# ska-telescope/ska-sdp-idg-bench

Hardware: AMD Instinct MI355X
Metric: Mvisibilities/s (gridder & degridder) at 1/2/4/8 GPUs; % HBM roofline (higher is better)
Workload: dtype f32 phase/accumulate, f16x2-split MFMA operands

## Files before the change

ska-sdp-idg-bench_amd/csrc/hip/kernels/gridder_mi355x.hip.cpp:

```cpp
#include <hip/hip_runtime.h>

#include <cstdlib>
#include <string>

#include "../util.hpp"
#include "device.hpp"
#include "fft.hpp"
#include "lib-hip.hpp"
#include "mfma.hpp"

#ifndef IDG_GRID_PT
#define IDG_GRID_PT 4
#endif
#ifndef IDG_GRID_WAVES
#define IDG_GRID_WAVES 4
#endif
#ifndef IDG_GRID_WAVES_GENERAL
#define IDG_GRID_WAVES_GENERAL 4
#endif
#ifndef IDG_GRID_BSCALE
#define IDG_GRID_BSCALE 12
#endif
#ifndef IDG_GRID_NW
#define IDG_GRID_NW 8
#endif

namespace idg_mi355x {

namespace {

__device__ __forceinline__ void mac4(float *a, const float4 &va,
                                     const float4 &vb, float cs, float sn) {
  a[0] = fma_(va.x, cs, a[0]); a[0] = fma_(-va.y, sn, a[0]);
  a[1] = fma_(va.x, sn, a[1]); a[1] = fma_(va.y, cs, a[1]);
  a[2] = fma_(va.z, cs, a[2]); a[2] = fma_(-va.w, sn, a[2]);
  a[3] = fma_(va.z, sn, a[3]); a[3] = fma_(va.w, cs, a[3]);
  a[4] = fma_(vb.x, cs, a[4]); a[4] = fma_(-vb.y, sn, a[4]);
  a[5] = fma_(vb.x, sn, a[5]); a[5] = fma_(vb.y, cs, a[5]);
  a[6] = fma_(vb.z, cs, a[6]); a[6] = fma_(-vb.w, sn, a[6]);
  a[7] = fma_(vb.z, sn, a[7]); a[7] = fma_(vb.w, cs, a[7]);
}

template <int NP, int CB>
__device__ __forceinline__ void timestep_general(
    const float (&l)[NP], const float (&m)[NP], const float (&n)[NP],
    const float (&poff)[NP], float (&acc)[NP][8],
    const idg::UVWCoordinate<float> c, const float4 *__restrict__ vrow,
    const float *__restrict__ wavenumbers, int C) {
  float pidx[NP];
#pragma unroll
  for (int i = 0; i < NP; ++i)
    pidx[i] = fma_(c.w, n[i], fma_(c.u, l[i], c.v * m[i]));
  for (int cb = 0; cb < C; cb += CB) {
    const int ce = min(cb + CB, C);
    const float k0 = wavenumbers[cb];
    float A[NP], R[NP];
#pragma unroll
    for (int i = 0; i < NP; ++i) {
      A[i] = fma_(-pidx[i], k0, poff[i]);
      R[i] = revolutions(A[i]);
    }
    float k = k0;
    float4 va = vrow[2 * cb], vb = vrow[2 * cb + 1];
    for (int ch = cb; ch < ce; ++ch) {
      const int nx = min(ch + 1, C - 1);
      const float kn = wavenumbers[nx];
      const float4 van = vrow[2 * nx], vbn = vrow[2 * nx + 1];
#pragma unroll
      for (int i = 0; i < NP; ++i) {
        const float ph = fma_(-pidx[i], k, poff[i]);
        const float r = fma_(ph - A[i], kInv2PiHi, R[i]);
        float sn, cs;
        sincos_rev(r, &sn, &cs);
        mac4(acc[i], va, vb, cs, sn);
      }
      k = kn;
      va = van;
      vb = vbn;
    }
  }
}

template <int NB, int CB>
__device__ __forceinline__ void timestep_mirror(
    const float (&l)[2 * NB], const float (&m)[2 * NB],
    const float (&poff)[2 * NB], float (&acc)[2 * NB][8],
    const idg::UVWCoordinate<float> c, const float4 *__restrict__ vrow,
    const float *__restrict__ wavenumbers, int C) {
  float pidx[NB];
#pragma unroll
  for (int i = 0; i < NB; ++i) pidx[i] = fma_(c.u, l[i], c.v * m[i]);
  for (int cb = 0; cb < C; cb += CB) {
    const int ce = min(cb + CB, C);
    const float k0 = wavenumbers[cb];
    float A[NB], R[NB];
#pragma unroll
    for (int i = 0; i < NB; ++i) {
      A[i] = fma_(-pidx[i], k0, poff[i]);
      R[i] = revolutions(A[i]);
    }
    float k = k0;
    float4 va = vrow[2 * cb], vb = vrow[2 * cb + 1];
    for (int ch = cb; ch < ce; ++ch) {
      const int nx = min(ch + 1, C - 1);
      const float kn = wavenumbers[nx];
      const float4 van = vrow[2 * nx], vbn = vrow[2 * nx + 1];
#pragma unroll
      for (int i = 0; i < NB; ++i) {
        const float ph = fma_(-pidx[i], k, poff[i]);
        const float r = fma_(ph - A[i], kInv2PiHi, R[i]);
        float sn, cs;
        sincos_rev(r, &sn, &cs);
        mac4(acc[i], va, vb, cs, sn);
        mac4(acc[NB + i], va, vb, cs, -sn);
      }
      k = kn;
      va = van;
      vb = vbn;
    }
  }
}

__device__ __forceinline__ void pixel_out(const float (&a)[8], int p, int S,
                                          const SubgridSetup &g,
                                          int nr_stations,
                                          const float *__restrict__ spheroidal,
                                          const float2 *__restrict__ aterms,
                                          float2 (&o)[4]) {
  const int y = p / S, x = p - (p / S) * S;
  idg::cfloat pix[4], a1[4], a2[4];
  for (int q = 0; q < 4; ++q) pix[q] = {a[2 * q], a[2 * q + 1]};
  load_jones(aterm_ptr(aterms, nr_stations, S, g.aterm_index, g.station1, y,
                       x), a1);
  load_jones(aterm_ptr(aterms, nr_stations, S, g.aterm_index, g.station2, y,
                       x), a2);
  idg::apply_aterm_gridder(pix, a1, a2);
  const float sph = spheroidal[p];
#pragma unroll
  for (int q = 0; q < 4; ++q) o[q] = make_float2(pix[q].re * sph, pix[q].im * sph);
}

__device__ __forceinline__ void store_pixel(
    const float (&a)[8], int p, int S, int npix, const SubgridSetup &g,
    int nr_stations, const float *__restrict__ spheroidal,
    const float2 *__restrict__ aterms, float2 *__restrict__ out) {
  float2 o[4];
  pixel_out(a, p, S, g, nr_stations, spheroidal, aterms, o);
#pragma unroll
  for (int q = 0; q < 4; ++q) out[static_cast<size_t>(q) * npix + p] = o[q];
}

template <bool W_TERMS = true>
__device__ __forceinline__ void pixel_geometry(int p, int S, float image_size,
                                               const SubgridSetup &g,
                                               float &l, float &m, float &n,
                                               float &poff) {
  const int y = p / S, x = p - (p / S) * S;
  l = idg::compute_l(x, S, image_size);
  m = idg::compute_m(y, S, image_size);
  if constexpr (W_TERMS) {
    n = idg::compute_n(l, m);
    poff = fma_(g.w_offset, n, fma_(g.u_offset, l, g.v_offset * m));
  } else {
    n = 0.0f;
    poff = fma_(g.u_offset, l, g.v_offset * m);
  }
}


#ifndef IDG_GRID_KSBUF
#define IDG_GRID_KSBUF 32
#endif
constexpr int kKsBuf = IDG_GRID_KSBUF;
#ifndef IDG_GRID_KSBUF_MIRROR
#define IDG_GRID_KSBUF_MIRROR (2 * IDG_GRID_KSBUF)
#endif
constexpr int kKsBufMirror = IDG_GRID_KSBUF_MIRROR;
#ifndef IDG_GRID_FILL_DEPTH
#define IDG_GRID_FILL_DEPTH 2
#endif
constexpr int mirror_fill_depth(int S_CT, bool combined) {
  return combined && S_CT != 32 ? 1 : IDG_GRID_FILL_DEPTH;
}

template <int AT, int NW>
struct MfmaLds {
  static constexpr int kObufFloats = NW * 16 * AT * 16;
  static constexpr int kBbufWords = kKsBuf * 64 * 8;
  static_assert(kKsBufMirror * 64 * 4 <= kBbufWords, "one buffer, two layouts");
  static constexpr int kUvwOff =
      kObufFloats > kBbufWords ? kObufFloats : kBbufWords;
  static constexpr int kRedOff = kUvwOff + 4 * 4 * kKsBuf;
  static constexpr int kSlotOff = kRedOff + 8;
  static constexpr int kSinkOff = kSlotOff + 2;
  static constexpr int kWords = kSinkOff + 64;
  static constexpr int kGeoOff = kWords;
  static constexpr int kWordsGeo = kGeoOff + 64 + 2 * 1024;
};
template <int S_CT, int NW, int AT>
constexpr int general_lds_words() {
  return S_CT == 32 ? MfmaLds<AT, NW>::kWordsGeo : MfmaLds<AT, NW>::kWords;
}

__device__ __forceinline__ void l2_prefetch_dma(const void *src,
                                                const void *lds_dst) {
  const unsigned m0 = __builtin_amdgcn_readfirstlane(static_cast<unsigned>(
      reinterpret_cast<size_t>((const __attribute__((address_space(3))) void *)
                                   lds_dst)));
  unsigned saved;
  asm volatile(
      "s_mov_b32 %0, m0\n\ts_mov_b32 m0, %2\n\ts_nop 0\n\t"
      "global_load_lds_dword %1, off\n\ts_mov_b32 m0, %0"
      : "=&s"(saved)
      : "v"(src), "s"(m0)
      : "memory");
}

template <int S_CT, int PT, int CB, int NW, bool MIRROR, bool FFT = false,
          int PREC = kPrecTail, bool PRESCAN = false,
          int FILL_D = IDG_GRID_FILL_DEPTH>
__device__ __forceinline__ void grid_mfma(
    const SubgridSetup &g, int S, int npix, float image_size, int C,
    int nr_stations, const idg::UVWCoordinate<float> *__restrict__ uvw,
    const float *__restrict__ wavenumbers,
    const float2 *__restrict__ visibilities,
    const float *__restrict__ spheroidal, const float2 *__restrict__ aterms,
    float2 *__restrict__ out, unsigned *lds, float vmax_pre = 0.0f,
    int pass_lo = 0, int pass_hi = 1 << 30) {
  static_assert(CB % 4 == 0, "anchor blocks hold whole channel quads");
  int tid = threadIdx.x;
  if constexpr (!MIRROR) asm volatile("" : "+v"(tid));
  const int lane = tid & 63, wave = tid >> 6;
  const int grp = lane >> 4, col = lane & 15;
  const int half = MIRROR ? npix / 2 : npix;
  constexpr bool kTailAlt = (PREC & kPrecTailAlt) != 0;
  constexpr bool kTailAll = (PREC & kPrecTail) != 0 && !kTailAlt;
  constexpr int AT = MIRROR ? 2 * PT : PT;
  using Lds = MfmaLds<AT, NW>;
  constexpr bool kGeoLds = !MIRROR && S_CT == 32;
  float *geo = reinterpret_cast<float *>(lds + Lds::kGeoOff);
  const int nt = g.nr_timesteps;
  const int nchq = (C + 3) / 4;
  const int nquads = (nt + 3) / 4;
  constexpr bool kOneFrag = MIRROR && S_CT != 0;
  constexpr int KS = kOneFrag ? kKsBufMirror : kKsBuf;
  const int quads_per_fill = nchq <= KS ? min(KS / nchq, kKsBuf) : 1;
  const int cq_per_fill = nchq <= KS ? nchq : KS;
  unsigned *slots = lds + Lds::kSlotOff;

  float vmax = vmax_pre;
  if (tid < 2) slots[tid] = 0u;
  if constexpr (!PRESCAN) {
    vmax = 0.0f;
    const float4 *v4 = reinterpret_cast<const float4 *>(
        visibilities + g.time_offset * C * 4);
    const int n4 = min(4 * quads_per_fill, nt) * C * 2;
    for (int i = tid; i < n4; i += NW * 64) {
      const float4 q = v4[i];
      vmax = fmaxf(vmax, fmaxf(fmaxf(fabsf(q.x), fabsf(q.y)),
                               fmaxf(fabsf(q.z), fabsf(q.w))));
    }
    for (int off = 32; off > 0; off >>= 1)
      vmax = fmaxf(vmax, __shfl_xor(vmax, off));
    float *red = reinterpret_cast<float *>(lds + Lds::kRedOff);
    if (lane == 0) red[wave] = vmax;
    __syncthreads();
#pragma unroll
    for (int w = 0; w < NW; ++w) vmax = fmaxf(vmax, red[w]);
  }
  constexpr int kBS = IDG_GRID_BSCALE;
  static_assert(kBS >= 0 && kBS <= 14, "a fill may reach 2^15 before it re-splits");
  int e = 0;
  bool have_scale = vmax > 0.0f && vmax <= 3.0e38f;
  if (have_scale) frexpf(vmax, &e);
  float scale = ldexpf(1.0f, kBS - e);
  int fidx = 0;

  const float2 *__restrict__ vsub = visibilities + g.time_offset * C * 4;

  uint4 *bbuf = reinterpret_cast<uint4 *>(lds);
  float *obuf = reinterpret_cast<float *>(lds);
  float4 *tuvw = reinterpret_cast<float4 *>(lds + Lds::kUvwOff);

  constexpr int kPass = NW * 16 * PT;
  for (int gbase = pass_lo; gbase < min(half, pass_hi); gbase += kPass) {
    static_assert(PT % 2 == 0, "phases are packed over tile pairs");
    constexpr int PH = PT / 2;
    floatx2 L2[PH], M2[PH], N2[PH], PG2[PH];
    if constexpr (kGeoLds) {
      static_assert(PT == 8 && NW == 8, "one S = 32 pass: 1,024 pixels");
      for (int p = tid; p < 1024; p += NW * 64) {
        float l, m, n, pg;
        pixel_geometry<true>(p, 32, image_size, g, l, m, n, pg);
        geo[64 + p] = n;
        geo[64 + 1024 + p] = pg;
        if (p < 32) geo[p] = l;
        if (p % 32 == 0) geo[32 + p / 32] = m;
      }
    } else {
#pragma unroll
      for (int i = 0; i < PT; ++i) {
        const int b = min(gbase + (wave * PT + i) * 16 + col, half - 1);
        float l, m, n, pg;
        pixel_geometry<!MIRROR>(b, S, image_size, g, l, m, n, pg);
        L2[i / 2][i % 2] = l;
        M2[i / 2][i % 2] = m;
        N2[i / 2][i % 2] = n;
        PG2[i / 2][i % 2] = pg;
      }
    }
    constexpr int PY = MIRROR ? PT : 1;
    floatx4 accx[PT], accy[PY];
#pragma unroll
    for (int i = 0; i < PT; ++i) accx[i] = floatx4{0.0f, 0.0f, 0.0f, 0.0f};
#pragma unroll
    for (int i = 0; i < PY; ++i) accy[i] = floatx4{0.0f, 0.0f, 0.0f, 0.0f};

    constexpr bool kFlush = (PREC & kPrecFlush) != 0;
    static_assert(!kFlush || S_CT == 32,
                  "the master fills the S = 32 output slot in one pass");
    bool flushed = false;
    auto master = [&](int t) {
      return reinterpret_cast<float4 *>(out) +
             ((wave * AT + t) * 32 + grp * 8 + (col & 7));
    };
    auto flush_tile = [&](floatx4 &a, int t, float unsc) {
      const float a0 = a[0], a1 = a[1], a2 = a[2], a3 = a[3];
      const float v0 = (a0 + row_ror8(a0)) * unsc;
      const float v1 = (a1 + row_ror8(a1)) * unsc;
      const float v2 = (a2 + row_ror8(a2)) * unsc;
      const float v3 = (a3 + row_ror8(a3)) * unsc;
      if (col < 8) {
        float4 m = make_float4(0.0f, 0.0f, 0.0f, 0.0f);
        if (flushed) m = *master(t);
        *master(t) = make_float4(m.x + v0, m.y + v1, m.z + v2, m.w + v3);
      }
      a = floatx4{0.0f, 0.0f, 0.0f, 0.0f};
    };

    for (int q0 = 0; q0 < nquads; q0 += quads_per_fill) {
      const int nq = min(quads_per_fill, nquads - q0);
      for (int j0 = 0; j0 < nchq; j0 += cq_per_fill, ++fidx) {
        const int nj = min(cq_per_fill, nchq - j0);
        for (;;) {
        __syncthreads();
        if (tid == 0) slots[(fidx + 1) & 1] = 0u;
        {
          const int bpol = (col & 7) >> 1;
          const int w_c = 2 * bpol + (col & 1);
          const int w_s = 2 * bpol + 1 - (col & 1);
          const float sc_s = (col & 1) ? scale : -scale;
          const float bpart = (col & 8) ? -1.0f : 0.0f;
          const float *vsubf = reinterpret_cast<const float *>(vsub);
          const int nks = nq * nj;
          const bool full = (q0 + nq) * 4 <= nt && 4 * (j0 + nj) <= C;
          const int wv = __builtin_amdgcn_readfirstlane(wave);
          const unsigned off_c = (grp * C * 8 + w_c) * 4u;
          const unsigned off_s = (grp * C * 8 + w_s) * 4u;
          int qq = wv / nj, jj = wv - (wv / nj) * nj;
          float lmax = 0.0f;
          if constexpr (kOneFrag) {
            auto load4 = [&](int q_, int j_, float (&b)[4]) {
              const int c0 = 4 * (j0 + j_);
              if (full) {
                const char *blk = reinterpret_cast<const char *>(
                    vsubf + ((q0 + q_) * 4 * C + c0) * 8);
#pragma unroll
                for (int u = 0; u < 4; ++u)
                  b[u] = *reinterpret_cast<const float *>(blk + off_c + 32 * u);
              } else {
                const int t = (q0 + q_) * 4 + grp;
#pragma unroll
                for (int u = 0; u < 4; ++u) {
                  const bool ok = t < nt && c0 + u < C;
                  b[u] = ok ? vsubf[(t * C + c0 + u) * 8 + w_c] : 0.0f;
                }
              }
            };
            auto put = [&](int ks, const float (&b)[4]) {
              lmax = fmaxf(lmax, fmaxf(fmaxf(fabsf(b[0]), fabsf(b[1])),
                                       fmaxf(fabsf(b[2]), fabsf(b[3]))));
              const unsigned xc =
                  split_part(b[0] * scale, b[1] * scale, bpart);
              const unsigned yc =
                  split_part(b[2] * scale, b[3] * scale, bpart);
              bbuf[ks * 64 + lane] = make_uint4(xc, xc, yc, yc);
            };
            auto advance = [&]() {
              jj += NW;
              while (jj >= nj) {
                jj -= nj;
                ++qq;
              }
            };
            constexpr int D = FILL_D;
            for (int ks = wv; ks < nks; ks += D * NW) {
              float b[D][4];
#pragma unroll
              for (int d = 0; d < D; ++d)
                if (ks + d * NW < nks) {
                  load4(qq, jj, b[d]);
                  advance();
                }
#pragma unroll
              for (int d = 0; d < D; ++d)
                if (ks + d * NW < nks) put(ks + d * NW, b[d]);
            }
          } else {
          for (int ks = wv; ks < nks; ks += NW) {
            const int t = (q0 + qq) * 4 + grp;
            const int c0 = 4 * (j0 + jj);
            float bc[4], bs[4];
            if (full) {
              const char *blk = reinterpret_cast<const char *>(
                  vsubf + ((q0 + qq) * 4 * C + c0) * 8);
#pragma unroll
              for (int u = 0; u < 4; ++u) {
                const float rc =
                    *reinterpret_cast<const float *>(blk + off_c + 32 * u);
                const float rs =
                    *reinterpret_cast<const float *>(blk + off_s + 32 * u);
                lmax = fmaxf(lmax, fmaxf(fabsf(rc), fabsf(rs)));
                bc[u] = rc * scale;
                bs[u] = rs * sc_s;
              }
            } else {
#pragma unroll
              for (int u = 0; u < 4; ++u) {
                const bool ok = t < nt && c0 + u < C;
                const int it = ok ? t * C + c0 + u : 0;
                const float rc = ok ? vsubf[it * 8 + w_c] : 0.0f;
                const float rs = ok ? vsubf[it * 8 + w_s] : 0.0f;
                lmax = fmaxf(lmax, fmaxf(fabsf(rc), fabsf(rs)));
                bc[u] = rc * scale;
                bs[u] = rs * sc_s;
              }
            }
            jj += NW;
            while (jj >= nj) {
              jj -= nj;
              ++qq;
            }
            const unsigned xc = split_part(bc[0], bc[1], bpart);
            const unsigned yc = split_part(bc[2], bc[3], bpart);
            const unsigned xs = split_part(bs[0], bs[1], bpart);
            const unsigned ys = split_part(bs[2], bs[3], bpart);
            bbuf[(ks * 64 + lane) * 2] = make_uint4(xc, xc, yc, yc);
            bbuf[(ks * 64 + lane) * 2 + 1] = make_uint4(xs, xs, ys, ys);
          }
          }
          {
            unsigned v = __float_as_uint(lmax);
            v = max(v, (unsigned)__builtin_amdgcn_update_dpp(0, (int)v, 0xB1, 0xF, 0xF, false));
            v = max(v, (unsigned)__builtin_amdgcn_update_dpp(0, (int)v, 0x4E, 0xF, 0xF, false));
            v = max(v, (unsigned)__builtin_amdgcn_update_dpp(0, (int)v, 0x124, 0xF, 0xF, false));
            v = max(v, (unsigned)__builtin_amdgcn_update_dpp(0, (int)v, 0x128, 0xF, 0xF, false));
            const unsigned wmax =
                max(max(__builtin_amdgcn_readlane(v, 0), __builtin_amdgcn_readlane(v, 16)),
                    max(__builtin_amdgcn_readlane(v, 32), __builtin_amdgcn_readlane(v, 48)));
            if (lane == 0) atomicMax(&slots[fidx & 1], wmax);
          }
          for (int i = tid; i < nq * 4; i += NW * 64) {
            const idg::UVWCoordinate<float> c =
                uvw[g.time_offset + min(q0 * 4 + i, nt - 1)];
            tuvw[i] = make_float4(c.u, c.v, c.w, 0.0f);
          }
        }
        __syncthreads();
        const float fm = __uint_as_float(
            __builtin_amdgcn_readfirstlane(slots[fidx & 1]));
        if (!(fm > 0.0f && fm <= 3.0e38f)) break;
        int em;
        frexpf(fm, &em);
        if (have_scale ? em <= e + 15 - kBS : em == e) {
          have_scale = true;
          break;
        }
        if (have_scale) {
          const float r = ldexpf(1.0f, e - em);
#pragma unroll
          for (int i = 0; i < PT; ++i) accx[i] *= r;
#pragma unroll
          for (int i = 0; i < PY; ++i) accy[i] *= r;
        }
        e = em;
        scale = ldexpf(1.0f, kBS - e);
        have_scale = true;
        }
        {
          int q0n = q0, j0n = j0 + cq_per_fill;
          if (j0n >= nchq) {
            j0n = 0;
            q0n = q0 + quads_per_fill;
          }
          if (q0n < nquads) {
            const int rows = min(4 * (q0n + quads_per_fill), nt) - 4 * q0n;
            const int lpr = (min(cq_per_fill, nchq - j0n) * 128 + 127) / 128;
            const char *vb = reinterpret_cast<const char *>(vsub);
            for (int ln = tid; ln < rows * lpr; ln += NW * 64) {
              const int row = ln / lpr, cl = ln - (ln / lpr) * lpr;
              l2_prefetch_dma(
                  vb + (static_cast<size_t>(4 * q0n + row) * C + 4 * j0n) * 32 +
                      cl * 128,
                  lds + Lds::kSinkOff);
            }
          }
        }
        for (int jb = 0; jb < nj; jb += CB / 4) {
          const int je = min(jb + CB / 4, nj);
          const float ka = wavenumbers[4 * (j0 + jb)];
          float kb[CB];
#pragma unroll
          for (int v = 0; v < CB; ++v)
            kb[v] = wavenumbers[min(4 * (j0 + jb) + v, C - 1)];
          for (int qq = 0; qq < nq; ++qq) {
            const float4 c4 = tuvw[qq * 4 + grp];
            const idg::UVWCoordinate<float> c = {c4.x, c4.y, c4.z};
            const floatx2 cu = {c.u, c.u}, cv = {c.v, c.v};
            const floatx2 ih = {kInv2PiHi, kInv2PiHi};
            if constexpr (!MIRROR) {
#pragma unroll
              for (int h = 0; h < PH; ++h) {
                if constexpr (kGeoLds) {
                  const int b0 = (wave * PT + 2 * h) * 16 + col;
                  L2[h] = floatx2{geo[col], geo[col + 16]};
                  const float mh = geo[32 + wave * (PT / 2) + h];
                  M2[h] = floatx2{mh, mh};
                  N2[h] = floatx2{geo[64 + b0], geo[64 + b0 + 16]};
                  PG2[h] = floatx2{geo[64 + 1024 + b0], geo[64 + 1024 + b0 + 16]};
                }
                floatx2 pidx = __builtin_elementwise_fma(cu, L2[h], cv * M2[h]);
                pidx = __builtin_elementwise_fma(floatx2{c.w, c.w}, N2[h], pidx);
                const floatx2 np = -pidx;
                const floatx2 a =
                    __builtin_elementwise_fma(np, floatx2{ka, ka}, PG2[h]);
                const floatx2 t = a * ih;
                const floatx2 nm = {-__builtin_rintf(t.x), -__builtin_rintf(t.y)};
                floatx2 cr = {0.0f, 0.0f};
                if constexpr (kTailAll) cr = tail_k_rev(np, ka);
                if constexpr (kTailAlt)
                  cr = tail_k_rev(np, 4.0f * ka);
#pragma unroll
                for (int u = 0; u < CB / 4; ++u) {
                  const int jj = jb + u;
                  if (jj >= je) break;
                  const int ks = qq * nj + jj;
                  const uint4 bx = bbuf[(ks * 64 + lane) * 2];
                  const uint4 by = bbuf[(ks * 64 + lane) * 2 + 1];
                  const half8 bfx = pack4(bx.x, bx.y, bx.z, bx.w);
                  const half8 bfy = pack4(by.x, by.y, by.z, by.w);
                  float snx[4], csx[4], sny[4], csy[4];
#pragma unroll
                  for (int j = 0; j < 4; ++j) {
                    const float kj = kb[4 * u + j];
                    const floatx2 ph =
                        __builtin_elementwise_fma(np, floatx2{kj, kj}, PG2[h]);
                    floatx2 r = __builtin_elementwise_fma(ph, ih, nm);
                    if constexpr (kTailAll) r = r + cr;
                    if constexpr (kTailAlt)
                      if (j == 0) r = r + cr;
                    sincos_rev(r.x, &snx[j], &csx[j]);
                    sincos_rev(r.y, &sny[j], &csy[j]);
                  }
                  half8 ac, as, ac1, as1;
                  split_oct(csx[0], csx[1], csx[2], csx[3], snx[0], snx[1],
                            snx[2], snx[3], &ac, &as);
                  split_oct(csy[0], csy[1], csy[2], csy[3], sny[0], sny[1],
                            sny[2], sny[3], &ac1, &as1);
                  accx[2 * h] = mfma16(ac, bfx, accx[2 * h]);
                  accx[2 * h + 1] = mfma16(ac1, bfx, accx[2 * h + 1]);
                  accx[2 * h] = mfma16(as, bfy, accx[2 * h]);
                  accx[2 * h + 1] = mfma16(as1, bfy, accx[2 * h + 1]);
                  IDG_KSTEP_FENCE();
                }
              }
              continue;
            }
            floatx2 NP[PH], NM[PH], CR[PH];
#pragma unroll
            for (int h = 0; h < PH; ++h) {
              const floatx2 pidx =
                  __builtin_elementwise_fma(cu, L2[h], cv * M2[h]);
              NP[h] = -pidx;
              const floatx2 a =
                  __builtin_elementwise_fma(NP[h], floatx2{ka, ka}, PG2[h]);
              const floatx2 t = a * ih;
              NM[h] = floatx2{-__builtin_rintf(t.x), -__builtin_rintf(t.y)};
              if constexpr (kTailAll)
                CR[h] = tail_k_rev(NP[h], ka);
              if constexpr (kTailAlt)
                CR[h] = tail_k_rev(NP[h], 4.0f * ka);
            }
#pragma unroll
            for (int u = 0; u < CB / 4; ++u) {
              const int jj = jb + u;
              if (jj >= je) break;
              const int ks = qq * nj + jj;
              const int fr = ks * 64 + lane;
              const uint4 bx = bbuf[kOneFrag ? fr : 2 * fr];
              const uint4 by = kOneFrag ? bx : bbuf[2 * fr + 1];
              const half8 bfx = pack4(bx.x, bx.y, bx.z, bx.w);
              const half8 bfy = pack4(by.x, by.y, by.z, by.w);
#pragma unroll
              for (int h = 0; h < PH; ++h) {
                float snx[4], csx[4], sny[4], csy[4];
#pragma unroll
                for (int j = 0; j < 4; ++j) {
                  const float kj = kb[4 * u + j];
                  const floatx2 ph =
                      __builtin_elementwise_fma(NP[h], floatx2{kj, kj}, PG2[h]);
                  floatx2 r = __builtin_elementwise_fma(ph, ih, NM[h]);
                  if constexpr (kTailAll) r = r + CR[h];
                  if constexpr (kTailAlt)
                    if (j == 0) r = r + CR[h];
                  sincos_rev(r.x, &snx[j], &csx[j]);
                  sincos_rev(r.y, &sny[j], &csy[j]);
                }
                half8 ac, as;
                split_oct(csx[0], csx[1], csx[2], csx[3], snx[0], snx[1],
                          snx[2], snx[3], &ac, &as);
                accx[2 * h] = mfma16(ac, bfx, accx[2 * h]);
                accy[2 * h] = mfma16(as, bfy, accy[2 * h]);
                split_oct(csy[0], csy[1], csy[2], csy[3], sny[0], sny[1],
                          sny[2], sny[3], &ac, &as);
                accx[2 * h + 1] = mfma16(ac, bfx, accx[2 * h + 1]);
                accy[2 * h + 1] = mfma16(as, bfy, accy[2 * h + 1]);
              }
              IDG_KSTEP_FENCE();
            }
          }
        }
        if constexpr (kFlush) {
          constexpr int kFlushEvery = kFlushFills * kKsBuf / KS;
          static_assert(kFlushEvery * KS == kFlushFills * kKsBuf,
                        "the flush period is a whole number of fills");
          const bool last =
              j0 + cq_per_fill >= nchq && q0 + quads_per_fill >= nquads;
          if (!last && (fidx + 1) % kFlushEvery == 0) {
            const float unsc = ldexpf(1.0f, e - kBS);
#pragma unroll
            for (int i = 0; i < PT; ++i) flush_tile(accx[i], i, unsc);
            if constexpr (MIRROR) {
#pragma unroll
              for (int i = 0; i < PY; ++i) flush_tile(accy[i], PT + i, unsc);
            }
            flushed = true;
          }
        }
      }
    }
    if constexpr (kFlush) {
      if (flushed && col < 8) {
        const float sc = ldexpf(1.0f, kBS - e);
#pragma unroll
        for (int i = 0; i < PT; ++i) {
          const float4 m = *master(i);
          accx[i] += floatx4{m.x, m.y, m.z, m.w} * sc;
        }
        if constexpr (MIRROR) {
#pragma unroll
          for (int i = 0; i < PY; ++i) {
            const float4 m = *master(PT + i);
            accy[i] += floatx4{m.x, m.y, m.z, m.w} * sc;
          }
        }
      }
    }

    const float unscale = ldexpf(1.0f, e - kBS);
    __syncthreads();
#pragma unroll
    for (int i = 0; i < PT; ++i)
#pragma unroll
      for (int r = 0; r < 4; ++r) {
        const int lp = (wave * PT + i) * 16 + grp * 4 + r;
        obuf[lp * 16 + col] = accx[i][r];
        if constexpr (MIRROR) obuf[(kPass + lp) * 16 + col] = accy[i][r];
      }
    __syncthreads();
    static_assert(!FFT || (S_CT == 32 && kPass >= (MIRROR ? 512 : 1024)),
                  "the FFT epilogue takes a whole S = 32 subgrid in one pass");
    constexpr int kIt = FFT ? kPass / (NW * 64) : 1;
    float2 keep[kIt][MIRROR ? 2 : 1][4];
    auto emit = [&](const float (&a)[8], int p, int it, int slot) {
      if constexpr (FFT)
        pixel_out(a, p, S, g, nr_stations, spheroidal, aterms, keep[it][slot]);
      else
        store_pixel(a, p, S, npix, g, nr_stations, spheroidal, aterms, out);
    };
    auto body = [&](int q, int it) {
      const int b = gbase + q;
      if (b >= half) return;
      const float4 *xr = reinterpret_cast<const float4 *>(obuf + q * 16);
      const float4 xh0 = xr[0], xh1 = xr[1], xl0 = xr[2], xl1 = xr[3];
      const float x[8] = {xh0.x + xl0.x, xh0.y + xl0.y, xh0.z + xl0.z,
                          xh0.w + xl0.w, xh1.x + xl1.x, xh1.y + xl1.y,
                          xh1.z + xl1.z, xh1.w + xl1.w};
      float y[8] = {0.0f, 0.0f, 0.0f, 0.0f, 0.0f, 0.0f, 0.0f, 0.0f};
      if constexpr (MIRROR) {
        const float4 *yr =
            reinterpret_cast<const float4 *>(obuf + (kPass + q) * 16);
        const float4 yh0 = yr[0], yh1 = yr[1], yl0 = yr[2], yl1 = yr[3];
        const float yv[8] = {yh0.x + yl0.x, yh0.y + yl0.y, yh0.z + yl0.z,
                             yh0.w + yl0.w, yh1.x + yl1.x, yh1.y + yl1.y,
                             yh1.z + yl1.z, yh1.w + yl1.w};
        if constexpr (kOneFrag) {
#pragma unroll
          for (int k = 0; k < 4; ++k) {
            y[2 * k] = -yv[2 * k + 1];
            y[2 * k + 1] = yv[2 * k];
          }
        } else {
#pragma unroll
          for (int j = 0; j < 8; ++j) y[j] = yv[j];
        }
      }
      float l, m, n, poff;
      pixel_geometry<!MIRROR>(b, S, image_size, g, l, m, n, poff);
      float tc, ts;
      phase_tail(poff, &tc, &ts);
      float ab[8];
#pragma unroll
      for (int j = 0; j < 8; ++j)
        ab[j] = (MIRROR ? x[j] + y[j] : x[j]) * unscale;
      rotate4(ab, tc, ts);
      emit(ab, b, it, 0);
      if constexpr (MIRROR) {
        float am[8];
#pragma unroll
        for (int j = 0; j < 8; ++j) am[j] = (x[j] - y[j]) * unscale;
        rotate4(am, tc, -ts);
        emit(am, npix - 1 - b, it, 1);
      }
    };
    if constexpr (FFT) {
#pragma unroll
      for (int it = 0; it < kIt; ++it) body(tid + it * NW * 64, it);
      constexpr int N = 32, RS = N + 1;
      float2 *planes = reinterpret_cast<float2 *>(lds);
      __syncthreads();
#pragma unroll
      for (int it = 0; it < kIt; ++it) {
        const int b = tid + it * NW * 64;
        if (b >= half) continue;
#pragma unroll
        for (int slot = 0; slot < (MIRROR ? 2 : 1); ++slot) {
          const int p = slot ? npix - 1 - b : b;
          const int row = p / N, col = p % N;
#pragma unroll
          for (int pol = 0; pol < 4; ++pol)
            planes[pol * N * RS + row * RS + col] = keep[it][slot][pol];
        }
      }
      __syncthreads();
      float2 tw[N / 2];
#pragma unroll
      for (int k = 0; k < N / 2; ++k) tw[k] = unit_phasor(k, N, 1.0f);
      float2 f[N];
      fft2_planes_lds<N>(planes, tid, 4 * N, tw, f);
      if (tid < 4 * N) {
        const int pp = tid / N, qq = tid % N;
#pragma unroll
        for (int i = 0; i < N; ++i)
          out[static_cast<size_t>(pp) * npix + bit_reverse<N>(i) * N + qq] =
              f[i];
      }
    } else {
      for (int q = tid; q < kPass; q += NW * 64) body(q, 0);
    }
    __syncthreads();
  }
}

template <int NW>
__device__ __forceinline__ bool prologue_scan(
    const SubgridSetup &g, int C,
    const idg::UVWCoordinate<float> *__restrict__ uvw,
    const float2 *__restrict__ visibilities, float *red) {
  const int tid = threadIdx.x;
  bool w_nonzero = false;
  for (int t = tid; t < g.nr_timesteps; t += NW * 64)
    w_nonzero |= uvw[g.time_offset + t].w != 0.0f;
  const int nchq = (C + 3) / 4;
  const int quads_per_fill = nchq <= kKsBuf ? kKsBuf / nchq : 1;
  const float4 *v4 = reinterpret_cast<const float4 *>(
      visibilities + g.time_offset * C * 4);
  const int n4 = min(4 * quads_per_fill, g.nr_timesteps) * C * 2;
  float vmax = 0.0f;
  for (int i = tid; i < n4; i += NW * 64) {
    const float4 q = v4[i];
    vmax = fmaxf(vmax, fmaxf(fmaxf(fabsf(q.x), fabsf(q.y)),
                             fmaxf(fabsf(q.z), fabsf(q.w))));
  }
  for (int off = 32; off > 0; off >>= 1)
    vmax = fmaxf(vmax, __shfl_xor(vmax, off));
  if ((tid & 63) == 0) red[tid >> 6] = vmax;
  return w_nonzero;
}

template <int NW>
__device__ __forceinline__ float prologue_max(const float *red) {
  float vmax = red[0];
#pragma unroll
  for (int w = 1; w < NW; ++w) vmax = fmaxf(vmax, red[w]);
  return vmax;
}

}

#if defined(IDG_WG_TIMELINE) && IDG_WG_TIMELINE
__device__ WgStamp idg_debug_timeline_gridder[kTimelineMax];
#endif

template <int S_CT, int PPT, int CB, int MODE, int PT, bool FFT = false,
          int PREC = kPrecTail>
__global__ void __launch_bounds__(MODE == 1 ? 64 * IDG_GRID_NW : kBlock,
                                  IDG_GRID_WAVES)
    kernel_gridder_mi355x(const int grid_size, int subgrid_size,
                          float image_size, float w_step_in_lambda,
                          int nr_channels, int nr_stations,
                          const idg::UVWCoordinate<float> *__restrict__ uvw,
                          const float *__restrict__ wavenumbers,
                          const float2 *__restrict__ visibilities,
                          const float *__restrict__ spheroidal,
                          const float2 *__restrict__ aterms,
                          const idg::Metadata *__restrict__ metadata,
                          float2 *__restrict__ subgrids) {
  static_assert(PPT % 2 == 0, "PPT must be even (pixel pairs)");
  constexpr int NB = PPT / 2;
  const int S = S_CT > 0 ? S_CT : subgrid_size;
  const int npix = S * S;
  const int s = xcd_subgrid(blockIdx.x, gridDim.x);
  const int tid = threadIdx.x;
  const SubgridSetup g = setup_subgrid(metadata, s, grid_size, S, image_size,
                                       w_step_in_lambda);
  const int C = nr_channels;
  float2 *out = subgrids + static_cast<size_t>(s) * 4 * npix;

  if constexpr (MODE == 1) {
    constexpr int NW = IDG_GRID_NW;
    __shared__ unsigned lds[general_lds_words<S_CT, NW, 2 * PT>()];
#if defined(IDG_WG_TIMELINE) && IDG_WG_TIMELINE
    timeline_start(idg_debug_timeline_gridder);
#endif
    float *red = reinterpret_cast<float *>(lds + MfmaLds<2 * PT, NW>::kRedOff);
    const bool mirror =
        __syncthreads_or(prologue_scan<NW>(g, C, uvw, visibilities, red)) ==
            0 &&
        S % 2 == 0 && g.w_offset == 0.0f;
    const float vmax = prologue_max<NW>(red);
    if (mirror)
      grid_mfma<S_CT, PT, CB, NW, true, FFT, PREC, true,
                mirror_fill_depth(S_CT, true)>(
          g, S, npix, image_size, C, nr_stations, uvw, wavenumbers,
          visibilities, spheroidal, aterms, out, lds, vmax);
    else
      grid_mfma<S_CT, 2 * PT, CB, NW, false, FFT, PREC, true>(
          g, S, npix, image_size, C, nr_stations, uvw, wavenumbers,
          visibilities, spheroidal, aterms, out, lds, vmax);
#if defined(IDG_WG_TIMELINE) && IDG_WG_TIMELINE
    timeline_end(idg_debug_timeline_gridder);
#endif
    return;
  }

  bool w_nonzero = false;
  for (int t = tid; t < g.nr_timesteps; t += blockDim.x)
    w_nonzero |= uvw[g.time_offset + t].w != 0.0f;
  const bool mirror = __syncthreads_or(w_nonzero) == 0 && S % 2 == 0 &&
                      g.w_offset == 0.0f;

  if (mirror) {
    const int half = npix / 2;
    for (int tile = 0; tile < half; tile += kBlock * NB) {
      float l[PPT], m[PPT], n[PPT], poff[PPT], acc[PPT][8];
#pragma unroll
      for (int i = 0; i < NB; ++i) {
        const int b = min(tile + i * kBlock + tid, half - 1);
        pixel_geometry(b, S, image_size, g, l[i], m[i], n[i], poff[i]);
        pixel_geometry(npix - 1 - b, S, image_size, g, l[NB + i], m[NB + i],
                       n[NB + i], poff[NB + i]);
      }
#pragma unroll
      for (int i = 0; i < PPT; ++i)
#pragma unroll
        for (int j = 0; j < 8; ++j) acc[i][j] = 0.0f;

      for (int t = 0; t < g.nr_timesteps; ++t) {
        const long long row = g.time_offset + t;
        const idg::UVWCoordinate<float> c = uvw[row];
        const float4 *vrow =
            reinterpret_cast<const float4 *>(visibilities + row * C * 4);
        timestep_mirror<NB, CB>(l, m, poff, acc, c, vrow, wavenumbers, C);
      }
#pragma unroll
      for (int i = 0; i < NB; ++i) {
        const int b = tile + i * kBlock + tid;
        if (b < half) {
          store_pixel(acc[i], b, S, npix, g, nr_stations, spheroidal, aterms,
                      out);
          store_pixel(acc[NB + i], npix - 1 - b, S, npix, g, nr_stations,
                      spheroidal, aterms, out);
        }
      }
    }
    return;
  }

  for (int tile = 0; tile < npix; tile += kBlock * PPT) {
    float l[PPT], m[PPT], n[PPT], poff[PPT], acc[PPT][8];
#pragma unroll
    for (int i = 0; i < PPT; ++i) {
      const int p = min(tile + i * kBlock + tid, npix - 1);
      pixel_geometry(p, S, image_size, g, l[i], m[i], n[i], poff[i]);
#pragma unroll
      for (int j = 0; j < 8; ++j) acc[i][j] = 0.0f;
    }
    for (int t = 0; t < g.nr_timesteps; ++t) {
      const long long row = g.time_offset + t;
      const idg::UVWCoordinate<float> c = uvw[row];
      const float4 *vrow =
          reinterpret_cast<const float4 *>(visibilities + row * C * 4);
      timestep_general<PPT, CB>(l, m, n, poff, acc, c, vrow, wavenumbers, C);
    }
#pragma unroll
    for (int i = 0; i < PPT; ++i) {
      const int p = tile + i * kBlock + tid;
      if (p < npix)
        store_pixel(acc[i], p, S, npix, g, nr_stations, spheroidal, aterms,
                    out);
    }
  }
}

template <int S_CT, int CB, int PT, bool FFT = false, int PREC = kPrecTail,
          int SPLIT = 1>
__global__ void __launch_bounds__(64 * IDG_GRID_NW, IDG_GRID_WAVES)
    kernel_gridder_mirror_mi355x(
        const int grid_size, int subgrid_size, float image_size,
        float w_step_in_lambda, int nr_channels, int nr_stations,
        const idg::UVWCoordinate<float> *__restrict__ uvw,
        const float *__restrict__ wavenumbers,
        const float2 *__restrict__ visibilities,
        const float *__restrict__ spheroidal,
        const float2 *__restrict__ aterms,
        const idg::Metadata *__restrict__ metadata,
        float2 *__restrict__ subgrids, int *__restrict__ queue) {
  constexpr int NW = IDG_GRID_NW;
  __shared__ unsigned lds[MfmaLds<2 * PT, NW>::kWords];
  const int S = S_CT > 0 ? S_CT : subgrid_size;
  const int npix = S * S;
  const int wg = xcd_subgrid(blockIdx.x, gridDim.x);
  const int s = SPLIT > 1 ? wg / SPLIT : wg;
  const int q = SPLIT > 1 ? wg % SPLIT : 0;
  const int tid = threadIdx.x;
  const SubgridSetup g = setup_subgrid(metadata, s, grid_size, S, image_size,
                                       w_step_in_lambda);
  float *red = reinterpret_cast<float *>(lds + MfmaLds<2 * PT, NW>::kRedOff);
  const bool mirror =
      __syncthreads_or(prologue_scan<NW>(g, nr_channels, uvw, visibilities,
                                         red)) == 0 &&
      S % 2 == 0 && g.w_offset == 0.0f;
  if (!mirror) {
    if constexpr (SPLIT > 1) {
      if (tid == 0 && q == 0)
        queue_push(queue, gridDim.x / SPLIT, s, s % kQueueShards);
    } else {
      if (tid == 0) queue_push(queue, gridDim.x, s);
    }
    return;
  }
  constexpr int kPass = NW * 16 * PT;
  static_assert(SPLIT == 1 || (S_CT > 0 && SPLIT * kPass >= S_CT * S_CT / 2 &&
                               (SPLIT - 1) * kPass < S_CT * S_CT / 2),
                "mirror_split(S) does not match the pass size");
  grid_mfma<S_CT, PT, CB, NW, true, FFT, PREC, true,
            mirror_fill_depth(S_CT, false)>(
      g, S, npix, image_size, nr_channels, nr_stations, uvw, wavenumbers,
      visibilities, spheroidal, aterms,
      subgrids + static_cast<size_t>(s) * 4 * npix, lds,
      prologue_max<NW>(red), SPLIT > 1 ? q * kPass : 0,
      SPLIT > 1 ? (q + 1) * kPass : 1 << 30);
}

template <int S_CT, int CB, int PT, bool FFT = false, int PREC = kPrecTail>
__global__ void __launch_bounds__(64 * IDG_GRID_NW, IDG_GRID_WAVES_GENERAL)
    kernel_gridder_general_mi355x(
        const int grid_size, int subgrid_size, float image_size,
        float w_step_in_lambda, int nr_channels, int nr_stations,
        const idg::UVWCoordinate<float> *__restrict__ uvw,
        const float *__restrict__ wavenumbers,
        const float2 *__restrict__ visibilities,
        const float *__restrict__ spheroidal,
        const float2 *__restrict__ aterms,
        const idg::Metadata *__restrict__ metadata,
        float2 *__restrict__ subgrids, int *__restrict__ queue,
        int nr_subgrids, int all) {
  constexpr int NW = IDG_GRID_NW;
  __shared__ unsigned lds[general_lds_words<S_CT, NW, 2 * PT>()];
  const int S = S_CT > 0 ? S_CT : subgrid_size;
  const int npix = S * S;
  const int tid = threadIdx.x;
  const QueueView qv = queue_view(queue, nr_subgrids);
  const int count = all ? nr_subgrids : qv.count();
  if (count == 0) return;
  if (tid == 0)
    lds[0] = static_cast<unsigned>(atomicAdd(queue + kQueueNext, 1));
  __syncthreads();
  int i = static_cast<int>(__builtin_amdgcn_readfirstlane(lds[0]));
  __syncthreads();
  while (i < count) {
    int next = 0;
    if (tid == 0) next = atomicAdd(queue + kQueueNext, 1);
    const int s = all ? i : qv.at(i);
    const SubgridSetup g = setup_subgrid(metadata, s, grid_size, S,
                                         image_size, w_step_in_lambda);
    grid_mfma<S_CT, 2 * PT, CB, NW, false, FFT, PREC>(
        g, S, npix, image_size, nr_channels, nr_stations, uvw, wavenumbers,
        visibilities, spheroidal, aterms,
        subgrids + static_cast<size_t>(s) * 4 * npix, lds);
    if (tid == 0) lds[0] = static_cast<unsigned>(next);
    __syncthreads();
    i = static_cast<int>(__builtin_amdgcn_readfirstlane(lds[0]));
    __syncthreads();
  }
  if (tid == 0) queue_retire(queue);
}

struct GridderSet {
  const void *combined, *mirror, *general;
};
constexpr int mirror_split(int S) { return S == 64 ? 4 : 1; }
template <int S_, int PPT_, bool FFT_, int PREC_>
GridderSet gridder_set() {
  return {reinterpret_cast<const void *>(
              &kernel_gridder_mi355x<S_, PPT_, 16, 1, IDG_GRID_PT, FFT_, PREC_>),
          reinterpret_cast<const void *>(
              &kernel_gridder_mirror_mi355x<S_, 16, IDG_GRID_PT, FFT_, PREC_,
                                            mirror_split(S_)>),
          reinterpret_cast<const void *>(
              &kernel_gridder_general_mi355x<S_, 16, IDG_GRID_PT, FFT_, PREC_>)};
}
template <int S_, int PPT_, bool FFT_>
GridderSet gridder_set_for(int prec) {
  if (prec & kPrecTailAlt) prec &= ~kPrecTail;
  if constexpr (S_ == 32) {
    switch (prec) {
      case 0: return gridder_set<S_, PPT_, FFT_, 0>();
      case kPrecTail | kPrecFlush:
        return gridder_set<S_, PPT_, FFT_, kPrecTail | kPrecFlush>();
      case kPrecFlush: return gridder_set<S_, PPT_, FFT_, kPrecFlush>();
      case kPrecTailAlt: return gridder_set<S_, PPT_, FFT_, kPrecTailAlt>();
      case kPrecTailAlt | kPrecFlush:
        return gridder_set<S_, PPT_, FFT_, kPrecTailAlt | kPrecFlush>();
      default: return gridder_set<S_, PPT_, FFT_, kPrecTail>();
    }
  } else {
    if (prec & kPrecTailAlt) return gridder_set<S_, PPT_, FFT_, kPrecTailAlt>();
    return (prec & kPrecTail) ? gridder_set<S_, PPT_, FFT_, kPrecTail>()
                              : gridder_set<S_, PPT_, FFT_, 0>();
  }
}
#define IDG_GRIDDER_VALU(S_, PPT_)                                        \
  reinterpret_cast<const void *>(                                         \
      &kernel_gridder_mi355x<S_, PPT_, 16, 0, IDG_GRID_PT>)

KernelChoice select_gridder(const Problem &p, const Options &request) {
  const Options opt = resolve_options(request);
  const int impl = opt.gridder_impl;
  KernelChoice k;
  k.grid = p.nr_subgrids;
  if (impl == kImplSequential) {
    k.func = sequential_gridder(p.subgrid_size);
    k.block = sequential_block();
    k.name = p.subgrid_size == 32   ? "gridder_sequential_mi355x_s32"
             : p.subgrid_size == 64 ? "gridder_sequential_mi355x_s64"
                                    : "gridder_sequential_mi355x_generic";
    return k;
  }
  if (impl == kImplOrdered) {
    k.func = ordered_gridder(p.subgrid_size);
    k.block = ordered_block();
    k.name = p.subgrid_size == 32   ? "gridder_ordered_mi355x_s32"
             : p.subgrid_size == 64 ? "gridder_ordered_mi355x_s64"
                                    : "gridder_ordered_mi355x_generic";
    return k;
  }
  const bool mfma = impl != kImplValu;
  const bool auto_ordered = impl == kImplAuto;
  k.auto_ordered = auto_ordered;
  k.auto_threshold = opt.auto_threshold;
  k.block = mfma ? 64 * IDG_GRID_NW : kBlock;
  k.prec = precision_for(Direction::kGridder, p, opt);
  if (k.prec & kPrecTailAlt) k.prec &= ~kPrecTail;
  if (p.subgrid_size != 32) k.prec &= ~kPrecFlush;
  if (!mfma) k.prec = 0;
  const bool fft_epilogue = p.fft_out && mfma && p.subgrid_size == 32 &&
                            !auto_ordered && opt.fft_fusion != kFftFusionOff;
  GridderSet set{};
  switch (p.subgrid_size) {
    case 32:
      set = fft_epilogue ? gridder_set_for<32, 4, true>(k.prec)
                         : gridder_set_for<32, 4, false>(k.prec);
      k.name = fft_epilogue ? "gridder_fft_mi355x_s32"
                            : (mfma ? "gridder_mi355x_s32"
                                    : "gridder_mi355x_s32_valu");
      k.fft_in_kernel = fft_epilogue;
      if (!mfma) set.combined = IDG_GRIDDER_VALU(32, 4);
      break;
    case 64:
      set = gridder_set_for<64, 4, false>(k.prec);
      k.name = mfma ? "gridder_mi355x_s64" : "gridder_mi355x_s64_valu";
      if (!mfma) set.combined = IDG_GRIDDER_VALU(64, 4);
      break;
    default:
      set = gridder_set_for<0, 2, false>(k.prec);
      k.name = mfma ? "gridder_mi355x_generic" : "gridder_mi355x_generic_valu";
      if (p.subgrid_size % 2 != 0) set.mirror = nullptr;
      if (!mfma) set.combined = IDG_GRIDDER_VALU(0, 2);
      break;
  }
  k.func = set.combined;
  if (auto_ordered)
    k.name = p.subgrid_size == 32   ? "gridder_auto_mi355x_s32"
             : p.subgrid_size == 64 ? "gridder_auto_mi355x_s64"
                                    : "gridder_auto_mi355x_generic";
  if (mfma && two_kernel_form(p.nr_subgrids, opt)) {
    if (set.mirror)
      k.parts[0] = {set.mirror, k.block, KernelChoice::kMirror,
                    mirror_split(p.subgrid_size)};
    k.parts[1] = {set.general, k.block, KernelChoice::kGeneral};
    k.all_general = {k.func, k.block, KernelChoice::kPlain};
  }
  return k;
}

}

namespace hip {

void p_run_gridder() {
  idg_mi355x::Problem p;
  p.subgrid_size = static_cast<int>(get_env_var("SUBGRID_SIZE", 32));
  p.nr_channels = static_cast<int>(get_env_var("NR_CHANNELS", 16));
  const idg_mi355x::KernelChoice k = idg_mi355x::select_gridder(p);
  p_run_gridder_(k.func, "gridder_mi355x", k.block);
}

void c_run_gridder(
    int nr_subgrids, int grid_size, int subgrid_size, float image_size,
    float w_step_in_lambda, int nr_channels, int nr_stations,
    idg::Array2D<idg::UVWCoordinate<float>> &uvw,
    idg::Array1D<float> &wavenumbers,
    idg::Array3D<idg::Visibility<std::complex<float>>> &visibilities,
    idg::Array2D<float> &spheroidal,
    idg::Array4D<idg::Matrix2x2<std::complex<float>>> &aterms,
    idg::Array1D<idg::Metadata> &metadata,
    idg::Array4D<std::complex<float>> &subgrids) {
  c_run_gridder_(nr_subgrids, grid_size, subgrid_size, image_size,
                 w_step_in_lambda, nr_channels, nr_stations, uvw, wavenumbers,
                 visibilities, spheroidal, aterms, metadata, subgrids, nullptr,
                 0);
}

}

#if defined(IDG_WG_TIMELINE) && IDG_WG_TIMELINE
extern "C" int idg_debug_timeline_gridder_copy(void *host, int n) {
  return hipMemcpyFromSymbol(
      host, HIP_SYMBOL(idg_mi355x::idg_debug_timeline_gridder),
      sizeof(WgStamp) * std::min(n, kTimelineMax));
}
#endif
```

Measured before the change: 3333.

## Pair k-slices per wave in mirror visibility fill and split hi/lo halves

In the one-fragment mirror fill path, each wave now handles two k-slices at once. Lanes 8-15 of each column group load the neighbouring channel block, so the loads are wider and more coalesced. The f16 hi/lo split is computed once per value with split_pair, and both halves go to separate LDS slots, replacing the per-lane bpart-selected split_part. The mirror fill depth also drops to 1 for non-FFT tight-precision variants, which trades load batching for lower register pressure.

```diff
diff --git a/ska-sdp-idg-bench_amd/csrc/hip/kernels/gridder_mi355x.hip.cpp b/ska-sdp-idg-bench_amd/csrc/hip/kernels/gridder_mi355x.hip.cpp
--- a/ska-sdp-idg-bench_amd/csrc/hip/kernels/gridder_mi355x.hip.cpp
+++ b/ska-sdp-idg-bench_amd/csrc/hip/kernels/gridder_mi355x.hip.cpp
@@ -179,8 +179,12 @@
 #ifndef IDG_GRID_FILL_DEPTH
 #define IDG_GRID_FILL_DEPTH 2
 #endif
-constexpr int mirror_fill_depth(int S_CT, bool combined) {
-  return combined && S_CT != 32 ? 1 : IDG_GRID_FILL_DEPTH;
+constexpr int mirror_fill_depth(int S_CT, bool combined, bool fft, int prec) {
+  const bool tight = prec == kPrecTail || prec == (kPrecTail | kPrecFlush) ||
+                     prec == (kPrecTailAlt | kPrecFlush);
+  return (combined && S_CT != 32) || (S_CT != 0 && !fft && tight)
+             ? 1
+             : IDG_GRID_FILL_DEPTH;
 }
 
 template <int AT, int NW>
@@ -360,19 +364,28 @@
           int qq = wv / nj, jj = wv - (wv / nj) * nj;
           float lmax = 0.0f;
           if constexpr (kOneFrag) {
+            const int hsel = col >> 3;
+            const bool paired = full && (nj & 1) == 0;
+            const unsigned off_p = off_c + 128u * hsel;
+            int qp = (2 * wv) / nj, jp = 2 * wv - ((2 * wv) / nj) * nj;
             auto load4 = [&](int q_, int j_, float (&b)[4]) {
-              const int c0 = 4 * (j0 + j_);
-              if (full) {
+              if (paired) {
                 const char *blk = reinterpret_cast<const char *>(
-                    vsubf + ((q0 + q_) * 4 * C + c0) * 8);
+                    vsubf + ((q0 + q_) * 4 * C + 4 * (j0 + j_)) * 8);
 #pragma unroll
                 for (int u = 0; u < 4; ++u)
-                  b[u] = *reinterpret_cast<const float *>(blk + off_c + 32 * u);
+                  b[u] = *reinterpret_cast<const float *>(blk + off_p + 32 * u);
               } else {
-                const int t = (q0 + q_) * 4 + grp;
+                int ql = q_, jl = j_ + hsel;
+                if (jl >= nj) {
+                  jl -= nj;
+                  ++ql;
+                }
+                const int t = (q0 + ql) * 4 + grp;
+                const int c0 = 4 * (j0 + jl);
 #pragma unroll
                 for (int u = 0; u < 4; ++u) {
-                  const bool ok = t < nt && c0 + u < C;
+                  const bool ok = ql < nq && t < nt && c0 + u < C;
                   b[u] = ok ? vsubf[(t * C + c0 + u) * 8 + w_c] : 0.0f;
                 }
               }
@@ -380,31 +393,34 @@
             auto put = [&](int ks, const float (&b)[4]) {
               lmax = fmaxf(lmax, fmaxf(fmaxf(fabsf(b[0]), fabsf(b[1])),
                                        fmaxf(fabsf(b[2]), fabsf(b[3]))));
-              const unsigned xc =
-                  split_part(b[0] * scale, b[1] * scale, bpart);
-              const unsigned yc =
-                  split_part(b[2] * scale, b[3] * scale, bpart);
-              bbuf[ks * 64 + lane] = make_uint4(xc, xc, yc, yc);
+              unsigned xh, xl, yh, yl;
+              split_pair(b[0] * scale, b[1] * scale, &xh, &xl);
+              split_pair(b[2] * scale, b[3] * scale, &yh, &yl);
+              if (ks + hsel < nks) {
+                uint4 *dst = bbuf + (ks + hsel) * 64 + grp * 16 + (col & 7);
+                dst[0] = make_uint4(xh, xh, yh, yh);
+                dst[8] = make_uint4(xl, xl, yl, yl);
+              }
             };
             auto advance = [&]() {
-              jj += NW;
-              while (jj >= nj) {
-                jj -= nj;
-                ++qq;
+              jp += 2 * NW;
+              while (jp >= nj) {
+                jp -= nj;
+                ++qp;
               }
             };
             constexpr int D = FILL_D;
-            for (int ks = wv; ks < nks; ks += D * NW) {
+            for (int ks = 2 * wv; ks < nks; ks += 2 * D * NW) {
               float b[D][4];
 #pragma unroll
               for (int d = 0; d < D; ++d)
-                if (ks + d * NW < nks) {
-                  load4(qq, jj, b[d]);
+                if (ks + 2 * d * NW < nks) {
+                  load4(qp, jp, b[d]);
                   advance();
                 }
 #pragma unroll
               for (int d = 0; d < D; ++d)
-                if (ks + d * NW < nks) put(ks + d * NW, b[d]);
+                if (ks + 2 * d * NW < nks) put(ks + 2 * d * NW, b[d]);
             }
           } else {
           for (int ks = wv; ks < nks; ks += NW) {
@@ -851,7 +867,7 @@
     const float vmax = prologue_max<NW>(red);
     if (mirror)
       grid_mfma<S_CT, PT, CB, NW, true, FFT, PREC, true,
-                mirror_fill_depth(S_CT, true)>(
+                mirror_fill_depth(S_CT, true, FFT, PREC)>(
           g, S, npix, image_size, C, nr_stations, uvw, wavenumbers,
           visibilities, spheroidal, aterms, out, lds, vmax);
     else
@@ -975,7 +991,7 @@
                                (SPLIT - 1) * kPass < S_CT * S_CT / 2),
                 "mirror_split(S) does not match the pass size");
   grid_mfma<S_CT, PT, CB, NW, true, FFT, PREC, true,
-            mirror_fill_depth(S_CT, false)>(
+            mirror_fill_depth(S_CT, false, FFT, PREC)>(
       g, S, npix, image_size, nr_channels, nr_stations, uvw, wavenumbers,
       visibilities, spheroidal, aterms,
       subgrids + static_cast<size_t>(s) * 4 * npix, lds,
```

New measurement: 3351, median of 6. No clear change (+0.6%).
